# StefanHeng/ECG-Representation-Learning

Measured on AMD Instinct MI355X. Metric: 12-lead ECG records/sec pre-train step, ViT-Base bf16 @ 1/2/4/8 MI355X, higher is better.
Workload: dtype bf16

## Files before the change

### ecg-representation-learning_amd/engine.py

```python
import math
from collections import OrderedDict

import os

import torch

from . import hip
from .hip import lib, check, ptr, stream, GEMM_NT, GEMM_NN, GEMM_TN
from .hip import EPI_BIAS, EPI_GELU, EPI_GELU_BWD, EPI_RESIDUAL, EPI_DROPOUT, EPI_COLSUM, EPI_GELU_GRAD_AUX, EPI_MUL_AUX

LN_EPS = 1e-5


def _align(n, a=8):
    return (n + a - 1) // a * a


def _numel(shape):
    n = 1
    for v in shape:
        n *= v
    return n


# ... 603 lines not shown

    def _act_spec(self, B, masked, m, rows=None, N=None, mrows=None):
        T = self.dtype
        f32, u8 = torch.float32, torch.uint8
        if N is None:
            N = self.n if masked else self.N
        M, Mp = B * N, B * (N if masked else N - 1)
        if rows is not None:
            M, Mp = rows, rows - (0 if masked else B)
        d, f, h = self.d, self.f, self.h
        sp = OrderedDict()
        sp.update(patches=((Mp, self.CP), T), tok=((Mp, d), T), x0=((M, d), T))
        for i in range(self.Ly):
            l = dict(mean1=((M,), f32), rstd1=((M,), f32), xn1=((M, d), T), qkv=((M, 3 * d), T), attn=((M, d), T), x1=((M, d), T),
                     mean2=((M,), f32), rstd2=((M,), f32), xn2=((M, d), T), hpre=((M, f), u8 if self._aux8(M) else T), hact=((M, f), T), x2=((M, d), T))
            if T == torch.float32:
                l['probs'] = ((B * h * N * N,), T)
            else:
                l['lse'] = ((B * h * N,), f32)
            if self.fp8 and M >= 2048:
                l.update(xn1_8=((M * d,), u8), attn_8=((M * d,), u8), xn2_8=((M * d,), u8), hact_8=((M * f,), u8))
            for k, v in l.items():
                sp[f'L{i}.{k}'] = v
        sp.update(logits=((B, self.K), f32), xhat=((B, d), f32), hrstd=((B,), f32), loss_elem=((B, self.K), f32), loss_mean=((1,), f32),
                  dlogits=((B, self.K), f32))
        sp.update(dxa=((M, d), T), dxb=((M, d), T), dxn=((M, d), T), dqkv=((M, 3 * d), T), dattn=((M, d), T), dh=((M, f), T),
                  dtok=((Mp, d), T), dxm=((M, d), T))
        if T == torch.float32:
            sp.update(pd=((B * h * N * N,), T), dp=((B * h * N * N,), T))
        if T == torch.bfloat16 and not masked:
            sp.update({f'cls_{k}': ((B, d), T) for k in ('attn', 'x1', 'xn2', 'x2', 'dx', 'dy', 'dxn', 'dx1', 'dxm', 'dattn', 'dq')})
            sp.update(cls_hpre=((B, f), T), cls_hact=((B, f), T), cls_dh=((B, f), T), cls_lse=((B * h,), f32), cls_mean2=((B,), f32),
                      cls_rstd2=((B,), f32))
        l = lib()
        ws = max(l.ecgvit_layernorm_bwd_workspace(M, d), l.ecgvit_colsum_workspace(M, max(f, 3 * d)), 8 * ((M + 255) // 256) * f, 4096)
        if T == torch.bfloat16:
            for (mm, nn) in ((d, f), (f, d), (d, d), (3 * d, d), (d, self.CP)):
                ws = max(ws, hip.gemm_workspace_bytes(GEMM_TN, T, mm, nn, M))
        if masked:
            Rm = B * m if mrows is None else mrows
            sp.update(flag=((Mp,), u8), rows=((Rm, d), T), pred=((Rm, self.CP), T), target=((Rm, self.CP), T),
                      dpred=((Rm, self.CP), T), drows=((Rm, d), T), dmasked=((Mp, d), T), mloss=((1,), f32), l1part=((1024,), f32))
        sp['ws'] = ((ws,), u8)
        if self.fp8:
            sp['q8'] = ((M * max(f, 3 * d),), u8)
            sp['q8b'] = ((M * f,), u8)
        return sp

    def _ln_fwd(self, x, g, b, y, mean, rstd, rows, q8_site=None, y8=None):
        d = self.d
        if (self.fp8 and q8_site is not None and q8_site in self._f8_seen and rows >= 2048 and d % 256 == 0
                and d // 64 in (4, 8, 12, 16, 24, 32)):
            check(lib().ecgvit_layernorm_fwd_q8(ptr(x), ptr(g), ptr(b), None if (y8 is not None and self._only8(rows)) else ptr(y), ptr(mean), ptr(rstd), rows, d, LN_EPS,
                                                ptr(y8 if y8 is not None else self.act['q8']),
                                                ptr(self.f8_scale[q8_site:q8_site + 1]), ptr(self.f8_amax[q8_site:q8_site + 1]), stream()),
                  'layernorm_fwd_q8')
            return True
        check(lib().ecgvit_layernorm_fwd(ptr(x), ptr(g), ptr(b), ptr(y), ptr(mean), ptr(rstd), rows, d, LN_EPS,
                                         hip.code(self.dtype), stream()), 'layernorm_fwd')
        return False

    def _ln_bwd(self, dy, x, g, mean, rstd, dres, dx, dg, db, rows):
        check(lib().ecgvit_layernorm_bwd(ptr(dy), ptr(x), ptr(g), ptr(mean), ptr(rstd), ptr(dres), ptr(dx), ptr(dg), ptr(db),
                                         ptr(self.act['ws']), rows, self.d, hip.code(self.dtype), stream()), 'layernorm_bwd')

    def _ln_bwd_fused(self, dy, x, g, mean, rstd, dres, dx, dg, db, rows, dxm, dcolsum, p, seed, q8_site=None):
# ... 152 lines not shown
                    and N * 3 * d * 2 < 2 ** 31):
                check(l.ecgvit_attention_bwd_q8(ptr(L['qkv']), ptr(L['attn']), ptr(a['dattn']), ptr(L['lse']), ptr(a['dqkv']), B, N, h, dh, self.scale,
                                                ph, seed, ptr(a['q8']), ptr(self.f8_scale[site:site + 1]), ptr(self.f8_amax[site:site + 1]), st),
                      'attention_bwd_q8')
                return True
            check(l.ecgvit_attention_bwd(ptr(L['qkv']), ptr(L['attn']), ptr(a['dattn']), ptr(L['lse']), ptr(a['dqkv']), B, N, h, dh, self.scale, ph,
                                         seed, hip.BF16, st), 'attention_bwd')
        else:
            self._attn_bwd_f32(L, B, ph, seed)
        return False

    def _attention_cls_fwd(self, L, B, ph, seed):
        a, l, st = self.act, lib(), stream()
        h, dh, N = self.h, self.dh, self.T
        ntok = self.saved.get('ntok')
        if ntok is not None:
            check(l.ecgvit_attention_varlen_cls_fwd(ptr(L['qkv']), ptr(a['cls_attn']), ptr(a['cls_lse']), ptr(ntok), B, N, h, dh, self.scale, ph, seed,
                                                    st), 'attention_varlen_cls_fwd')
        else:
            check(l.ecgvit_attention_cls_fwd(ptr(L['qkv']), ptr(a['cls_attn']), ptr(a['cls_lse']), B, N, h, dh, self.scale, ph, seed,
                                             hip.code(self.dtype), st), 'attention_cls_fwd')

    def _attention_cls_bwd(self, L, B, ph, seed):
        a, l, st = self.act, lib(), stream()
        h, dh, N = self.h, self.dh, self.T
        ntok = self.saved.get('ntok')
        if ntok is not None:
            check(l.ecgvit_attention_varlen_cls_bwd(ptr(L['qkv']), ptr(a['cls_attn']), ptr(a['cls_dattn']), ptr(a['cls_lse']), ptr(a['dqkv']),
                                                    ptr(a['cls_dq']), ptr(ntok), B, N, h, dh, self.scale, ph, seed, st), 'attention_varlen_cls_bwd')
        else:
            check(l.ecgvit_attention_cls_bwd(ptr(L['qkv']), ptr(a['cls_attn']), ptr(a['cls_dattn']), ptr(a['cls_lse']), ptr(a['dqkv']), ptr(a['cls_dq']),
                                             B, N, h, dh, self.scale, ph, seed, hip.code(self.dtype), st), 'attention_cls_bwd')

    def _cls_block_fwd(self, L, X, B, ph, s0, lp):
        a, W, P = self.act, self.W, self.P32
        d, f, N = self.d, self.f, self.T
        M = B * N
        self._ln_fwd(X, P[lp + '0.norm.weight'], P[lp + '0.norm.bias'], L['xn1'], L['mean1'], L['rstd1'], M)
        wqkv = W[lp + '0.fn.to_qkv.weight']
        self._gemm(GEMM_NT, L['xn1'], wqkv, L['qkv'], M, 2 * d, d, d, d, 3 * d, b_off=d * d, c_off=d)
        self._gemm(GEMM_NT, L['xn1'], wqkv, L['qkv'], B, d, d, N * d, d, N * 3 * d)
        self._attention_cls_fwd(L, B, ph, s0 + 1)
        drop = EPI_DROPOUT if ph > 0 else 0
        self._gemm(GEMM_NT, a['cls_attn'], W[lp + '0.fn.to_out.0.weight'], a['cls_x1'], B, d, d, d, d, d, epilogue=EPI_BIAS | EPI_RESIDUAL | drop,
                   bias=P[lp + '0.fn.to_out.0.bias'], residual=X, ldr=N * d, dropout_p=ph, seed=s0 + 2, mask_row_pitch=N)
        self._ln_fwd(a['cls_x1'], P[lp + '1.norm.weight'], P[lp + '1.norm.bias'], a['cls_xn2'], a['cls_mean2'], a['cls_rstd2'], B)
        self._gemm(GEMM_NT, a['cls_xn2'], W[lp + '1.fn.net.0.weight'], a['cls_hact'], B, f, d, d, d, f,
                   epilogue=EPI_BIAS | EPI_GELU | EPI_GELU_GRAD_AUX | drop, bias=P[lp + '1.fn.net.0.bias'], aux=a['cls_hpre'], ldaux=f,
                   dropout_p=ph, seed=s0 + 3, mask_row_pitch=N)
        self._gemm(GEMM_NT, a['cls_hact'], W[lp + '1.fn.net.3.weight'], a['cls_x2'], B, d, f, f, f, d, epilogue=EPI_BIAS | EPI_RESIDUAL | drop,
                   bias=P[lp + '1.fn.net.3.bias'], residual=a['cls_x1'], ldr=d, dropout_p=ph, seed=s0 + 4, mask_row_pitch=N)
        return a['cls_x2']

    def forward(self, x, labels=None, weight=None, training=True, seed=0, want_mean=True, cls_only_last=False, lengths=None):
        return self._head_loss(self._trunk_pass(x, labels, weight, training, seed, cls_only_last, lengths), want_mean)

    def _head_loss(self, X, want_mean):
        a, sv, T = self.act, self.saved, hip.code(self.dtype)
        l, st = lib(), stream()
        B, d, rg, labels = sv['B'], self.d, sv['ragged'], sv['labels']
        pre = 'vit.'
        sv['head_pitch'] = 1 if (sv['cls_only_last'] or rg is not None) else self.N
        if rg is not None:
            check(l.ecgvit_gather_rows(ptr(X), ptr(rg.tok_off), ptr(a['cls_x2']), 1, rg.M, B, d, d, d, T, st), 'gather_rows')
            X = a['cls_x2']
        check(l.ecgvit_head_fwd(ptr(X), sv['head_pitch'], ptr(self.P32[pre + 'mlp_head.0.weight']), ptr(self.P32[pre + 'mlp_head.0.bias']),
                                ptr(self.P32[pre + 'mlp_head.1.weight']), ptr(self.P32[pre + 'mlp_head.1.bias']),
                                ptr(a['logits']), ptr(a['xhat']), ptr(a['hrstd']), B, d, self.K, LN_EPS, T, st), 'head_fwd')
        if labels is None:
            return a['logits'], None, None
        check(l.ecgvit_bce_fwd(ptr(a['logits']), ptr(labels), ptr(sv['weight']), ptr(a['loss_elem']),
                               ptr(a['loss_mean']) if want_mean else None, B * self.K, st), 'bce_fwd')
        return a['logits'], a['loss_elem'], (a['loss_mean'] if want_mean else None)

    def _trunk_pass(self, x, labels, weight, training, seed, cls_only_last, lengths):
# ... 448 lines not shown
        s0 = seed + 100 * (i + 1)
        Xin = a['x0'] if i == 0 else a['layers'][i - 1]['x2']
        dY = dXc
        if ph > 0:
            check(l.ecgvit_dropout_apply_rows(ptr(dXc), ptr(a['cls_dy']), B, d, N, ph, s0 + 4, T, st), 'dropout_apply_rows')
            dY = a['cls_dy']
        self._colsum(dY, d, G[lp + '1.fn.net.3.bias'], B, d)
        if self._wants(lp + '1.fn.net.3.weight'):
            self._gemm(GEMM_TN, dY, a['cls_hact'], G[lp + '1.fn.net.3.weight'], d, f, B, d, f, f, workspace=ws)
        b = self._stage(i, 0)
        if not self._reach(b):
            return None, None
        self._gemm(GEMM_NN, dY, W[lp + '1.fn.net.3.weight'], a['cls_dh'], B, f, d, d, f, f, epilogue=EPI_MUL_AUX | EPI_COLSUM, aux=a['cls_hpre'],
                   ldaux=f, workspace=ws, colsum_out=G[lp + '1.fn.net.0.bias'])
        if self._wants(lp + '1.fn.net.0.weight'):
            self._gemm(GEMM_TN, a['cls_dh'], a['cls_xn2'], G[lp + '1.fn.net.0.weight'], f, d, B, f, d, d, workspace=ws)
        if not self._reach(b + 1):
            return None, None
        self._gemm(GEMM_NN, a['cls_dh'], W[lp + '1.fn.net.0.weight'], a['cls_dxn'], B, d, f, f, d, d)
        if not self._reach(b + 2):
            return None, None
        check(l.ecgvit_layernorm_bwd_fused_rowpitch(ptr(a['cls_dxn']), ptr(a['cls_x1']), ptr(P[lp + '1.norm.weight']), ptr(a['cls_mean2']),
                                                    ptr(a['cls_rstd2']), ptr(dXc), ptr(a['cls_dx1']), ptr(G[lp + '1.norm.weight']),
                                                    ptr(G[lp + '1.norm.bias']), ptr(ws), B, d, ptr(a['cls_dxm']), ptr(G[lp + '0.fn.to_out.0.bias']),
                                                    ph, s0 + 2, N, T, st), 'layernorm_bwd_fused_rowpitch')
        dY = a['cls_dxm'] if ph > 0 else a['cls_dx1']
        if self._wants(lp + '0.fn.to_out.0.weight'):
            self._gemm(GEMM_TN, dY, a['cls_attn'], G[lp + '0.fn.to_out.0.weight'], d, d, B, d, d, d, workspace=ws)
        if not self._reach(b + 3):
            return None, None
        self._gemm(GEMM_NN, dY, W[lp + '0.fn.to_out.0.weight'], a['cls_dattn'], B, d, d, d, d, d)
        if not self._reach(b + 4):
            return None, None
        self._attention_cls_bwd(L, B, ph, s0 + 1)
        name = lp + '0.fn.to_qkv.weight'
        if self._wants(name):
            self._gemm(GEMM_TN, a['dqkv'], L['xn1'], G[name], 2 * d, d, M, 3 * d, d, d, workspace=ws, a_off=d, c_off=d * d)
            self._gemm(GEMM_TN, a['cls_dq'], L['xn1'], G[name], d, d, B, d, N * d, d, workspace=ws)
        if not self._reach(b + 5):
            return None, None
        wt = self.WT.get(name)
        if wt is not None and M >= 2048:
            self._gemm(GEMM_NT, a['dqkv'], wt, a['dxn'], M, d, 2 * d, 3 * d, 3 * d, d, a_off=d, b_off=d)
        else:
            self._gemm(GEMM_NN, a['dqkv'], W[name], a['dxn'], M, d, 2 * d, 3 * d, d, d, a_off=d, b_off=d * d)
        self._gemm(GEMM_NN, a['cls_dq'], W[name], a['dxn'], B, d, d, d, d, N * d, epilogue=hip.EPI_ACCUM)
        if not self._reach(b + 6):
            return None, None
        dres.zero_()
        check(l.ecgvit_scatter_rows(ptr(a['cls_dx1']), ptr(self._cls_rows(B)), ptr(dres), B, N, 1, d, d, d, T, st), 'scatter_rows')
        if i > 0:
            lq = f'vit.transformer.layers.{i - 1}.'
            self._ln_bwd_fused(a['dxn'], Xin, P[lp + '0.norm.weight'], L['mean1'], L['rstd1'], dres, out, G[lp + '0.norm.weight'],
                               G[lp + '0.norm.bias'], M, a['dxm'], G[lq + '1.fn.net.3.bias'], ph, seed + 100 * i + 4)
        else:
            self._ln_bwd(a['dxn'], Xin, P[lp + '0.norm.weight'], L['mean1'], L['rstd1'], dres, out, G[lp + '0.norm.weight'], G[lp + '0.norm.bias'], M)
        self._ready(f'layer{i}')
        return out, dres

    def _cls_rows(self, B):
        t = getattr(self, '_cls_idx', None)
        if t is None or t.numel() < B or t.device != self.device:
            t = self._cls_idx = torch.zeros(max(B, 1), dtype=torch.int32, device=self.device)
        return t[:B]

    def _attn_bwd_f32(self, L, B, ph, seed):
        d, h, dh, N = self.d, self.h, self.dh, self.T
        a = self.act
        qkv, P, dqkv, dO, dP = L['qkv'], L['probs'], a['dqkv'], a['dattn'], a['dp']
        sq, so, sp = (N * 3 * d, dh), (N * d, dh), (h * N * N, N * N)
        Pd = P
        if ph > 0:
            Pd = a['pd']
            self._drop_apply_f32(P, Pd, B * h * N * N, ph, seed)
        self._gemm(GEMM_TN, Pd, dO, dqkv, N, dh, N, N, d, 3 * d, batch=(B, h), strideA=sp, strideB=so, strideC=sq, c_off=2 * d)
# ... 65 lines not shown
```

### ecg-representation-learning_amd/hip.py

```python
import ctypes
import os
from ctypes import c_int, c_int32, c_int64, c_uint64, c_float, c_double, c_void_p, c_char_p, POINTER, Structure, byref

import torch

_PKG_DIR = os.path.dirname(os.path.abspath(__file__))
LIB_PATH = os.path.join(_PKG_DIR, 'libecgvit_hip.so')

ABI_VERSION = 6
F32, BF16, FP8_E4M3, BF8_E5M2 = 0, 1, 2, 3
GEMM_NT, GEMM_NN, GEMM_TN = 0, 1, 2
EPI_BIAS, EPI_GELU, EPI_GELU_BWD, EPI_RESIDUAL, EPI_ACCUM, EPI_DROPOUT, EPI_COLSUM = 1, 2, 4, 8, 16, 32, 64
EPI_GELU_GRAD_AUX, EPI_MUL_AUX, EPI_QUANT_OUT, EPI_NO_OUT, EPI_AUX8 = 128, 256, 512, 1024, 2048

ACC_INIT, ACC_ADD, ACC_FOLD = 0, 1, 2
KERNEL_NONE, KERNEL_GEMM_F32, KERNEL_GEMM_BF16, KERNEL_GEMM_NT, KERNEL_GEMM_WGRAD = 0, 1, 2, 3, 4
POOL_CLS, POOL_MEAN = 0, 1
FIT_TARGETS, FIT_BINS = 16, 256
DENOISE_MAX_LEN, DENOISE_MAX_TAPS = 32768, 9
DENOISE_MAX_LEN_TILED = 1 << 25
DENOISE_MAX_POINTS = 1024

_ERR = {1: 'ECGVIT_EINVAL (unsupported shape / argument)', 2: 'ECGVIT_ELAUNCH (HIP launch failure)'}

# ... 81 lines not shown
    'ecgvit_cast_bf16_to_f32': (c_int, [_P, _P, _L, _P]),
    'ecgvit_transpose_bf16_batched': (c_int, [_P, _P, _P, _I, _L, _P]),
    'ecgvit_mask_embed_finish': (c_int, [_P, _P, _P, _P, _P, _P, _I, _I, _I, _I, _I, _P]),
    'ecgvit_mask_embed_bwd': (c_int, [_P, _P, _P, _P, _P, _I, _I, _I, _I, _P]),
    'ecgvit_mask_embed_varlen_fwd': (c_int, [_P, _P, _P, _P, _P, _P, _P, _P, _I, _I, _I, _L, _I, _I, _I, _P]),
    'ecgvit_mask_embed_varlen_bwd': (c_int, [_P, _P, _P, _P, _P, _P, _P, _P, _I, _I, _I, _I, _I, _P]),
    'ecgvit_gather_rows': (c_int, [_P, _P, _P, _I, _I, _I, _L, _L, _L, _I, _P]),
    'ecgvit_scatter_rows': (c_int, [_P, _P, _P, _I, _I, _I, _L, _L, _L, _I, _P]),
    'ecgvit_l1_loss_fwd_bwd': (c_int, [_P, _P, _P, _P, _P, _P, _L, _I, _L, _I, _P]),
    'ecgvit_eval_counts': (c_int, [_P, _L, _P, _L, _L, _I, _I, _I, _P, _P]),
    'ecgvit_pool_records': (c_int, [_P, _P, _P, _P, _I, _I, _I, _I, _P, _P, _F, _I, _P]),
    'ecgvit_rollout_workspace': (c_int64, [_I, _I, _I]),
    'ecgvit_rollout_cls': (c_int, [_P, _P, _P, _P, _P, _P, _I, _I, _I, _I, _F, _I, _P]),
    'ecgvit_rollout_colsum': (c_int, [_P, _P, _P, _P, _P, _P, _P, _P, _I, _I, _I, _I, _F, _I, _P]),
    'ecgvit_rollout_finish': (c_int, [_P, _P, _I, _I, _I, _P]),
    'ecgvit_fit_workspace': (c_int64, [_I, _I]),
    'ecgvit_fit_moments': (c_int, [_P, _P, _L, _P, _I, _I, _P, _P, _P, _P]),
    'ecgvit_fit_histogram': (c_int, [_P, _P, _L, _P, _I, _I, _P, _I, _I, _P, _P]),
    'ecgvit_fit_select': (c_int, [_P, _P, _I, _I, _I, _P]),
    'ecgvit_tok_assign': (c_int, [_P, _P, _L, _P, _P, _P, _L, _I, _I, _L, _I, _I, _P, _I, _P, _P, _P, _P, _P, _P]),
    'ecgvit_tok_workspace': (c_int64, [_I, _I]),
    'ecgvit_tok_update': (c_int, [_P, _P, _L, _P, _P, _P, _L, _I, _I, _L, _I, _I, _P, _P, _I, _P, _P, _I, _P]),
    'ecgvit_tok_decode': (c_int, [_P, _P, _L, _P, _P, _P, _L, _I, _I, _L, _I, _P, _P, _P, _I, _P]),
    'ecgvit_denoise_workspace': (c_int64, [_I, _I, _I]),
    'ecgvit_filtfilt': (c_int, [_P, _P, _P, _L, _P, _I, _I, _I, _I, POINTER(c_double), POINTER(c_double), POINTER(c_double), _I, _P, _P]),
    'ecgvit_nlm_sigma': (c_int, [_P, _P, _L, _P, _I, _I, _I, _P, _P, _P]),
    'ecgvit_nlm_denoise': (c_int, [_P, _P, _P, _L, _P, _I, _I, _I, _P, _D, _I, _I, _P]),
    'ecgvit_rloess': (c_int, [_P, _P, _P, _L, _P, _I, _I, _I, _I, _I, _D, _I, _I, _I, _P, _P]),
    'ecgvit_denoise_workspace_long': (c_int64, [_I, _I, _I]),
    'ecgvit_filtfilt_long': (c_int, [_P, _P, _P, _L, _P, _I, _I, _I, _I, POINTER(c_double), POINTER(c_double), POINTER(c_double), _I, _P, _P]),
    'ecgvit_nlm_sigma_long': (c_int, [_P, _P, _L, _P, _I, _I, _I, _P, _P, _P]),
    'ecgvit_nlm_denoise_tiled': (c_int, [_P, _P, _P, _L, _P, _I, _I, _I, _P, _D, _I, _I, _I, _P]),
    'ecgvit_rloess_tiled': (c_int, [_P, _P, _P, _L, _P, _I, _I, _I, _I, _I, _D, _I, _I, _I, _P, _I, _P]),
}

_lib = None


def use_library(path):
    global LIB_PATH
    if _lib is not None:
        raise RuntimeError('use_library() must come before the first ecgvit call of the process')
    if not os.path.exists(path):
        raise HipLibraryMissing(f'{path} not found')
    LIB_PATH = os.path.abspath(path)


def lib():
    global _lib
    if _lib is None:
        if not os.path.exists(LIB_PATH):
            raise HipLibraryMissing(
                f'{LIB_PATH} not found: build it with `python -c "import __graft_entry__ as g; g.build()"` '
                f'(or `make -C {os.path.join(_PKG_DIR, "csrc")}`). There is no CPU / eager fallback.')
        l = ctypes.CDLL(LIB_PATH)
        for name, (res, args) in SIGNATURES.items():
            fn = getattr(l, name)
            fn.restype, fn.argtypes = res, args
        _lib = l
    return _lib


def check(rc, what):
    if rc != 0:
        raise RuntimeError(f'{what}: {_ERR.get(rc, rc)}')

# ... 68 lines not shown
```

### include/ecgvit_hip.h

```cpp
#ifndef ECGVIT_HIP_H
#define ECGVIT_HIP_H

#include <stdint.h>

#ifdef __cplusplus
extern "C" {
#endif

#define ECGVIT_OK 0
#define ECGVIT_EINVAL 1
#define ECGVIT_ELAUNCH 2

#define ECGVIT_F32 0
#define ECGVIT_BF16 1
#define ECGVIT_FP8_E4M3 2
#define ECGVIT_BF8_E5M2 3

const char *ecgvit_version(void);
int ecgvit_abi_version(void);

#define ECGVIT_GEMM_NT 0
#define ECGVIT_GEMM_NN 1
#define ECGVIT_GEMM_TN 2

// ... 202 lines not shown

int ecgvit_tok_assign(const float *x, const int64_t *src_off, int64_t lead_stride, const int32_t *raw_len, const int64_t *seg_cum,
                      const int64_t *dst_off, int64_t dst_stride, int R, int C, int64_t n_seg, int k, int pad, const float *centers, int V,
                      const int32_t *prev_ids, int32_t *ids, float *means, float *dist, uint64_t *changed, void *stream);
int64_t ecgvit_tok_workspace(int V, int k);
int ecgvit_tok_update(const float *x, const int64_t *src_off, int64_t lead_stride, const int32_t *raw_len, const int64_t *seg_cum,
                      const int64_t *dst_off, int64_t dst_stride, int R, int C, int64_t n_seg, int k, int pad, const int32_t *ids,
                      float *centers, int V, int64_t *lens, void *workspace, int keep_amax, void *stream);
int ecgvit_tok_decode(float *out, const int64_t *src_off, int64_t lead_stride, const int32_t *raw_len, const int64_t *seg_cum,
                      const int64_t *dst_off, int64_t dst_stride, int R, int C, int64_t n_seg, int k, const int32_t *ids, const float *means,
                      const float *centers, int V, void *stream);

int64_t ecgvit_denoise_workspace(int R, int C, int max_len);
int ecgvit_filtfilt(const float *x, float *out, const int64_t *src_off, int64_t lead_stride, const int32_t *raw_len, int R, int C, int min_len,
                    int max_len, const double *b, const double *a, const double *zi, int ntaps, void *workspace, void *stream);
int ecgvit_nlm_sigma(const float *x, const int64_t *src_off, int64_t lead_stride, const int32_t *raw_len, int R, int C, int max_len, double *sigma,
                     void *workspace, void *stream);
int ecgvit_nlm_denoise(const float *x, float *out, const int64_t *src_off, int64_t lead_stride, const int32_t *raw_len, int R, int C, int max_len,
                       const double *sigma, double scale, int patch_wd, int sch_wd, void *stream);
int ecgvit_rloess(const float *x, float *out, const int64_t *src_off, int64_t lead_stride, const int32_t *raw_len, int R, int C, int min_len,
                  int max_len, int npoints, double frac, int degree, int robust_iters, int subtract, int8_t *iters, void *stream);

int64_t ecgvit_denoise_workspace_long(int R, int C, int max_len);
int ecgvit_filtfilt_long(const float *x, float *out, const int64_t *src_off, int64_t lead_stride, const int32_t *raw_len, int R, int C, int min_len,
                         int max_len, const double *b, const double *a, const double *zi, int ntaps, void *workspace, void *stream);
int ecgvit_nlm_sigma_long(const float *x, const int64_t *src_off, int64_t lead_stride, const int32_t *raw_len, int R, int C, int max_len, double *sigma,
                          void *workspace, void *stream);
int ecgvit_nlm_denoise_tiled(const float *x, float *out, const int64_t *src_off, int64_t lead_stride, const int32_t *raw_len, int R, int C, int max_len,
                             const double *sigma, double scale, int patch_wd, int sch_wd, int tile_runs, void *stream);
int ecgvit_rloess_tiled(const float *x, float *out, const int64_t *src_off, int64_t lead_stride, const int32_t *raw_len, int R, int C, int min_len,
                        int max_len, int npoints, double frac, int degree, int robust_iters, int subtract, int8_t *iters, int tile_samples,
                        void *stream);

#ifdef __cplusplus
}
#endif
#endif
```

Measured before the change: 7110.

## Fold CLS-only last-layer K/V projections into query-side vectors to skip full K/V GEMMs

When only the CLS token is needed in the last block, the K and V projections over all tokens are no longer computed. Instead, each head's query is folded through Wk into a vector u, scores are taken directly against the normed inputs, probabilities weight the input rows, and Wv is applied afterward. The backward pass is folded the same way, and dedicated kernels compute the K/V weight gradients. This removes an M x 2d x d GEMM in the forward pass and its matching backward GEMMs, at the cost of custom fp32 MFMA kernels, extra fp32 buffers and a possible change in numerics.

```diff
diff --git a/ecg-representation-learning_amd/csrc/cls_kv_fold.hip b/ecg-representation-learning_amd/csrc/cls_kv_fold.hip
--- /dev/null
+++ b/ecg-representation-learning_amd/csrc/cls_kv_fold.hip
@@ -0,0 +1,425 @@
+#include "common.h"
+
+namespace {
+
+constexpr int CF_MAX_N = 2048;
+constexpr int CF_MAX_H = 12;
+constexpr int CF_LDS_BYTES = 64 * 1024;
+
+__host__ __device__ inline int cf_pitch(int N) {
+    const int np = (N + 15) & ~15;
+    return (np & 31) ? np : np + 16;
+}
+static inline int cf_strips(int d) { return d / 128; }
+static inline int cf_parts(int d) { return 12 / cf_strips(d); }
+
+static bool cf_shape_ok(int N, int h, int d) {
+    if (N < 1 || N > CF_MAX_N || h < 2 || h > CF_MAX_H || (h & 1) || d != 64 * h) return false;
+    return ((int64_t)h * d + 2ll * h * cf_pitch(N)) * 4 <= CF_LDS_BYTES;
+}
+
+template <bool DROP> __device__ __forceinline__ float cf_mult(uint32_t smix, uint32_t quad0, int key, uint32_t thresh, float inv_keep) {
+    if constexpr (!DROP) return 1.f;
+    const uint32_t hsh = quad_hash(smix, quad0 + (uint32_t)(key >> 2));
+    return ((hsh >> (8 * (key & 3))) & 0xFFu) >= thresh ? inv_keep : 0.f;
+}
+
+__device__ __forceinline__ f32x4 cf_mfma(float a, float b, f32x4 c) { return __builtin_amdgcn_mfma_f32_16x16x4f32(a, b, c, 0, 0, 0); }
+__device__ __forceinline__ f32x4 cf_ld4(const float *p) { return *reinterpret_cast<const f32x4 *>(p); }
+__device__ __forceinline__ void cf_st4(float *p, f32x4 v) { *reinterpret_cast<f32x4 *>(p) = v; }
+__device__ __forceinline__ void cf_unpack(u32x4 raw, float (&v)[8]) {
+#pragma unroll
+    for (int i = 0; i < 4; ++i) {
+        v[2 * i] = __uint_as_float(raw[i] << 16);
+        v[2 * i + 1] = __uint_as_float(raw[i] & 0xFFFF0000u);
+    }
+}
+
+__device__ __forceinline__ void cf_fill_frags(float *frag, const float *__restrict__ u, int h, int d) {
+    const int d4 = d >> 2;
+    for (int i = threadIdx.x; i < h * d4; i += blockDim.x) {
+        const int n = i / d4, q = i - n * d4;
+        cf_st4(frag + ((int64_t)q * h + n) * 4, cf_ld4(u + (int64_t)n * d + 4 * q));
+    }
+}
+
+__device__ __forceinline__ void cf_scores(const bf16_t *__restrict__ y, const float *frag, float *out, int np, int N, int h, int d, float mul,
+                                          int wave, int nwaves, int lane) {
+    const int r = lane & 15, kq = lane >> 4;
+    const int nn = min(r, h - 1);
+    const int steps = d >> 5;
+    for (int t = wave; t * 16 < N; t += nwaves) {
+        const bf16_t *yr = y + (int64_t)min(t * 16 + r, N - 1) * d + 8 * kq;
+        f32x4 acc = {0.f, 0.f, 0.f, 0.f};
+        u32x4 raw[4];
+#pragma unroll
+        for (int p = 0; p < 4; ++p) raw[p] = *reinterpret_cast<const u32x4 *>(yr + 32 * p);
+        for (int s = 0; s < steps; s += 4) {
+#pragma unroll
+            for (int p = 0; p < 4; ++p) {
+                const u32x4 cur = raw[p];
+                if (s + p + 4 < steps) raw[p] = *reinterpret_cast<const u32x4 *>(yr + 32 * (s + p + 4));
+                const float *fb = frag + ((int64_t)(8 * (s + p) + 2 * kq) * h + nn) * 4;
+                const f32x4 b0 = cf_ld4(fb), b1 = cf_ld4(fb + 4 * h);
+                float a[8];
+                cf_unpack(cur, a);
+#pragma unroll
+                for (int i = 0; i < 4; ++i) acc = cf_mfma(a[i], b0[i], acc);
+#pragma unroll
+                for (int i = 0; i < 4; ++i) acc = cf_mfma(a[4 + i], b1[i], acc);
+            }
+        }
+#pragma unroll
+        for (int g = 0; g < 4; ++g) {
+            const int j = t * 16 + kq * 4 + g;
+            if (r < h && j < N) out[r * np + j] = acc[g] * mul;
+        }
+    }
+}
+
+__device__ __forceinline__ void cf_weighted_rows(const bf16_t *__restrict__ y, const float *coef, int np, float *red, float *__restrict__ dst, int N,
+                                                 int h, int d, int strip, int part, int parts, int lane) {
+    const int n = lane & 15, kq = lane >> 4;
+    const int c0 = strip * 128 + 8 * n;
+    const float *ca = coef + min(n, h - 1) * np + kq;
+    const int nsteps = (N + 3) >> 2;
+    f32x4 acc[8];
+#pragma unroll
+    for (int i = 0; i < 8; ++i) acc[i] = f32x4{0.f, 0.f, 0.f, 0.f};
+    auto load = [&](int s) -> u32x4 {
+        const int row = 4 * s + kq;
+        return row < N ? *reinterpret_cast<const u32x4 *>(y + (int64_t)row * d + c0) : u32x4{0u, 0u, 0u, 0u};
+    };
+    u32x4 raw[4];
+#pragma unroll
+    for (int p = 0; p < 4; ++p) raw[p] = part + p * parts < nsteps ? load(part + p * parts) : u32x4{0u, 0u, 0u, 0u};
+    for (int s0 = part; s0 < nsteps; s0 += 4 * parts) {
+#pragma unroll
+        for (int p = 0; p < 4; ++p) {
+            const int s = s0 + p * parts;
+            if (s < nsteps) {
+                const u32x4 cur = raw[p];
+                if (s + 4 * parts < nsteps) raw[p] = load(s + 4 * parts);
+                const float a = ca[4 * s];
+                float v[8];
+                cf_unpack(cur, v);
+#pragma unroll
+                for (int i = 0; i < 8; ++i) acc[i] = cf_mfma(a, v[i], acc[i]);
+            }
+        }
+    }
+    for (int p = 0; p < parts; ++p) {
+        if (part == p) {
+#pragma unroll
+            for (int g = 0; g < 4; ++g) {
+                const int head = kq * 4 + g;
+                if (head < h) {
+                    f32x4 v0 = {acc[0][g], acc[1][g], acc[2][g], acc[3][g]}, v1 = {acc[4][g], acc[5][g], acc[6][g], acc[7][g]};
+                    float *rp = red + head * d + c0;
+                    if (p > 0) {
+                        v0 = cf_ld4(rp) + v0;
+                        v1 = cf_ld4(rp + 4) + v1;
+                    }
+                    if (p == parts - 1) {
+                        cf_st4(dst + (int64_t)head * d + c0, v0);
+                        cf_st4(dst + (int64_t)head * d + c0 + 4, v1);
+                    } else {
+                        cf_st4(rp, v0);
+                        cf_st4(rp + 4, v1);
+                    }
+                }
+            }
+        }
+        __syncthreads();
+    }
+}
+
+template <bool DROP>
+__global__ __launch_bounds__(768) void cls_fold_fwd_kernel(const bf16_t *__restrict__ xn, const float *__restrict__ u, float *__restrict__ probs,
+                                                          float *__restrict__ t, int N, int h, int d, int parts, float scale, uint64_t seed,
+                                                          uint32_t thresh, float inv_keep) {
+    extern __shared__ __attribute__((aligned(16))) float cf_smem[];
+    const int np = cf_pitch(N);
+    float *frag = cf_smem, *sc = cf_smem + h * d;
+    const int b = blockIdx.x;
+    const int lane = threadIdx.x & 63, wave = __builtin_amdgcn_readfirstlane(threadIdx.x >> 6), nwaves = blockDim.x >> 6;
+    const bf16_t *y = xn + (int64_t)b * N * d;
+    cf_fill_frags(frag, u + (int64_t)b * h * d, h, d);
+    __syncthreads();
+    cf_scores(y, frag, sc, np, N, h, d, scale, wave, nwaves, lane);
+    __syncthreads();
+    const uint32_t smix = seed_mix(seed);
+    for (int head = wave; head < h; head += nwaves) {
+        float *s = sc + head * np;
+        float m = -INFINITY;
+        for (int j = lane; j < N; j += 64) m = fmaxf(m, s[j]);
+        m = wave_max(m);
+        float sum = 0.f;
+        for (int j = lane; j < N; j += 64) sum += __expf(s[j] - m);
+        const float l = m + __logf(wave_sum(sum));
+        const uint32_t quad0 = (uint32_t)(b * h + head) * (uint32_t)N * (uint32_t)((N + 3) >> 2);
+        float *pr = probs + ((int64_t)b * h + head) * N;
+        for (int j = lane; j < np; j += 64) {
+            float pd = 0.f;
+            if (j < N) {
+                const float p = __expf(s[j] - l);
+                pr[j] = p;
+                pd = p * cf_mult<DROP>(smix, quad0, j, thresh, inv_keep);
+            }
+            s[j] = pd;
+        }
+    }
+    __syncthreads();
+    cf_weighted_rows(y, sc, np, frag, t + (int64_t)b * h * d, N, h, d, wave % (d >> 7), wave / (d >> 7), parts, lane);
+}
+
+template <bool DROP>
+__global__ __launch_bounds__(768) void cls_fold_bwd_kernel(const bf16_t *__restrict__ xn, const float *__restrict__ u, const float *__restrict__ w,
+                                                          const float *__restrict__ probs, float *__restrict__ z, bf16_t *__restrict__ dxn, int N,
+                                                          int h, int d, int parts, float scale, uint64_t seed, uint32_t thresh, float inv_keep) {
+    extern __shared__ __attribute__((aligned(16))) float cf_smem[];
+    const int np = cf_pitch(N);
+    float *frag = cf_smem, *coef = cf_smem + h * d;
+    const int b = blockIdx.x;
+    const int lane = threadIdx.x & 63, wave = __builtin_amdgcn_readfirstlane(threadIdx.x >> 6), nwaves = blockDim.x >> 6;
+    const bf16_t *y = xn + (int64_t)b * N * d;
+    const float *ub = u + (int64_t)b * h * d, *wb = w + (int64_t)b * h * d;
+    cf_fill_frags(frag, wb, h, d);
+    __syncthreads();
+    cf_scores(y, frag, coef, np, N, h, d, 1.0f, wave, nwaves, lane);
+    __syncthreads();
+    const uint32_t smix = seed_mix(seed);
+    for (int head = wave; head < h; head += nwaves) {
+        float *dp = coef + head * np, *pdr = coef + (h + head) * np;
+        const float *pr = probs + ((int64_t)b * h + head) * N;
+        const uint32_t quad0 = (uint32_t)(b * h + head) * (uint32_t)N * (uint32_t)((N + 3) >> 2);
+        float D = 0.f;
+        for (int j = lane; j < N; j += 64) D = fmaf(pr[j] * cf_mult<DROP>(smix, quad0, j, thresh, inv_keep), dp[j], D);
+        D = wave_sum(D);
+        for (int j = lane; j < np; j += 64) {
+            float ds = 0.f, pd = 0.f;
+            if (j < N) {
+                const float p = pr[j], mlt = cf_mult<DROP>(smix, quad0, j, thresh, inv_keep);
+                pd = p * mlt;
+                ds = scale * p * (dp[j] * mlt - D);
+            }
+            dp[j] = ds;
+            pdr[j] = pd;
+        }
+    }
+    __syncthreads();
+    const int strips = d >> 7, strip = wave % strips, part = wave / strips;
+    cf_weighted_rows(y, coef, np, frag, z + (int64_t)b * h * d, N, h, d, strip, part, parts, lane);
+    if (dxn == nullptr) return;
+    const int n = lane & 15, kq = lane >> 4, ksteps = h >> 1;
+    const int c0 = strip * 128 + 8 * n;
+    f32x4 bf[CF_MAX_H / 2][2];
+#pragma unroll
+    for (int ks = 0; ks < CF_MAX_H / 2; ++ks) {
+        bf[ks][0] = bf[ks][1] = f32x4{0.f, 0.f, 0.f, 0.f};
+        if (ks < ksteps) {
+            const int kk = 4 * ks + kq;
+            const float *src = (kk < h ? ub + (int64_t)kk * d : wb + (int64_t)(kk - h) * d) + c0;
+            bf[ks][0] = cf_ld4(src);
+            bf[ks][1] = cf_ld4(src + 4);
+        }
+    }
+    bf16_t *dy = dxn + (int64_t)b * N * d + c0;
+    for (int t = part; t * 16 < N; t += parts) {
+        f32x4 acc[8];
+#pragma unroll
+        for (int i = 0; i < 8; ++i) acc[i] = f32x4{0.f, 0.f, 0.f, 0.f};
+#pragma unroll
+        for (int ks = 0; ks < CF_MAX_H / 2; ++ks) {
+            if (ks < ksteps) {
+                const float a = coef[(4 * ks + kq) * np + t * 16 + n];
+#pragma unroll
+                for (int i = 0; i < 8; ++i) acc[i] = cf_mfma(a, bf[ks][i >> 2][i & 3], acc[i]);
+            }
+        }
+#pragma unroll
+        for (int g = 0; g < 4; ++g) {
+            const int row = t * 16 + kq * 4 + g;
+            if (row < N) {
+                bf16x8 o;
+#pragma unroll
+                for (int i = 0; i < 8; ++i) o[i] = (bf16_t)acc[i][g];
+                *reinterpret_cast<bf16x8 *>(dy + (int64_t)row * d) = o;
+            }
+        }
+    }
+}
+
+__global__ __launch_bounds__(128) void cls_fold_vec_kernel(const bf16_t *__restrict__ x, int64_t ldx, const bf16_t *__restrict__ W,
+                                                          float *__restrict__ out, int B, int h, int d) {
+    __shared__ __attribute__((aligned(16))) float xs[64][16];
+    const int head = blockIdx.y, b0 = blockIdx.z * 16, c = blockIdx.x * 256 + 2 * threadIdx.x;
+    for (int i = threadIdx.x; i < 1024; i += 128) {
+        const int bb = i >> 6, e = i & 63;
+        xs[e][bb] = b0 + bb < B ? (float)x[(int64_t)(b0 + bb) * ldx + 64 * head + e] : 0.f;
+    }
+    __syncthreads();
+    if (c >= d) return;
+    float a0[16], a1[16];
+#pragma unroll
+    for (int k = 0; k < 16; ++k) a0[k] = a1[k] = 0.f;
+    const bf16_t *wp = W + (int64_t)64 * head * d + c;
+#pragma unroll 4
+    for (int e = 0; e < 64; ++e) {
+        const bf16x2 wv = *reinterpret_cast<const bf16x2 *>(wp + (int64_t)e * d);
+        const float w0 = (float)wv[0], w1 = (float)wv[1];
+#pragma unroll
+        for (int q = 0; q < 4; ++q) {
+            const f32x4 xv = cf_ld4(&xs[e][4 * q]);
+#pragma unroll
+            for (int k = 0; k < 4; ++k) {
+                a0[4 * q + k] = fmaf(xv[k], w0, a0[4 * q + k]);
+                a1[4 * q + k] = fmaf(xv[k], w1, a1[4 * q + k]);
+            }
+        }
+    }
+#pragma unroll
+    for (int k = 0; k < 16; ++k)
+        if (b0 + k < B) *reinterpret_cast<f32x2 *>(out + ((int64_t)(b0 + k) * h + head) * d + c) = f32x2{a0[k], a1[k]};
+}
+
+__global__ __launch_bounds__(256) void cls_fold_head_kernel(const float *__restrict__ v, const bf16_t *__restrict__ W, bf16_t *__restrict__ out,
+                                                           int64_t ldo, int B, int h, int d) {
+    extern __shared__ __attribute__((aligned(16))) float cf_smem[];
+    const int head = blockIdx.x, b0 = blockIdx.y * 16, d4 = d >> 2;
+    for (int i = threadIdx.x; i < 16 * d4; i += 256) {
+        const int bb = i / d4, q = i - bb * d4;
+        cf_st4(cf_smem + bb * d + 4 * q, b0 + bb < B ? cf_ld4(v + ((int64_t)(b0 + bb) * h + head) * d + 4 * q) : f32x4{0.f, 0.f, 0.f, 0.f});
+    }
+    __syncthreads();
+    const int e = threadIdx.x & 63, wv = threadIdx.x >> 6;
+    const bf16_t *wp = W + (int64_t)(64 * head + e) * d;
+    float acc[4] = {0.f, 0.f, 0.f, 0.f};
+#pragma unroll 2
+    for (int c = 0; c < d; c += 8) {
+        float wf[8];
+        cf_unpack(*reinterpret_cast<const u32x4 *>(wp + c), wf);
+#pragma unroll
+        for (int k = 0; k < 4; ++k) {
+            const float *tp = cf_smem + (4 * wv + k) * d + c;
+            const f32x4 t0 = cf_ld4(tp), t1 = cf_ld4(tp + 4);
+#pragma unroll
+            for (int i = 0; i < 4; ++i) acc[k] = fmaf(wf[i], t0[i], acc[k]);
+#pragma unroll
+            for (int i = 0; i < 4; ++i) acc[k] = fmaf(wf[4 + i], t1[i], acc[k]);
+        }
+    }
+#pragma unroll
+    for (int k = 0; k < 4; ++k)
+        if (b0 + 4 * wv + k < B) out[(int64_t)(b0 + 4 * wv + k) * ldo + 64 * head + e] = (bf16_t)acc[k];
+}
+
+__global__ __launch_bounds__(512) void cls_fold_wgrad_kernel(const bf16_t *__restrict__ xk, int64_t ldk, const float *__restrict__ vk,
+                                                            float *__restrict__ dWk, const bf16_t *__restrict__ xv, int64_t ldv,
+                                                            const float *__restrict__ vv, float *__restrict__ dWv, int B, int h, int d) {
+    __shared__ float red[16][64];
+    const bool vside = blockIdx.z >= 4;
+    const bf16_t *x = vside ? xv : xk;
+    const int64_t ldx = vside ? ldv : ldk;
+    const float *v = vside ? vv : vk;
+    float *dW = vside ? dWv : dWk;
+    const int head = blockIdx.y, e0 = 16 * (blockIdx.z & 3), lane = threadIdx.x & 63, c = blockIdx.x * 64 + lane;
+    const int wave = __builtin_amdgcn_readfirstlane(threadIdx.x >> 6);
+    float acc[16];
+#pragma unroll
+    for (int k = 0; k < 16; ++k) acc[k] = 0.f;
+#pragma unroll 4
+    for (int b = wave; b < B; b += 8) {
+        const float vc = v[((int64_t)b * h + head) * d + c];
+        const bf16_t *xp = x + (int64_t)b * ldx + 64 * head + e0;
+        float xf[16];
+        cf_unpack(*reinterpret_cast<const u32x4 *>(xp), *reinterpret_cast<float(*)[8]>(xf));
+        cf_unpack(*reinterpret_cast<const u32x4 *>(xp + 8), *reinterpret_cast<float(*)[8]>(xf + 8));
+#pragma unroll
+        for (int k = 0; k < 16; ++k) acc[k] = fmaf(xf[k], vc, acc[k]);
+    }
+    for (int p = 0; p < 8; ++p) {
+        if (wave == p) {
+#pragma unroll
+            for (int k = 0; k < 16; ++k) {
+                const float s = p > 0 ? red[k][lane] + acc[k] : acc[k];
+                if (p == 7) dW[(int64_t)(64 * head + e0 + k) * d + c] = s;
+                else red[k][lane] = s;
+            }
+        }
+        __syncthreads();
+    }
+}
+
+static bool cf_aligned16(const void *p) { return reinterpret_cast<uintptr_t>(p) % 16 == 0; }
+
+}
+
+extern "C" {
+
+int ecgvit_cls_fold_supported(int N, int h, int d) { return cf_shape_ok(N, h, d) ? 1 : 0; }
+
+int ecgvit_cls_fold_vec(const void *x, int64_t ldx, const void *W, float *out, int B, int h, int d, void *stream) {
+    if (!x || !W || !out || B < 1 || h < 1 || d != 64 * h || ldx < d || (B + 15) / 16 > 65535 || h > 65535) return ECGVIT_EINVAL;
+    hipLaunchKernelGGL(cls_fold_vec_kernel, dim3((unsigned)((d + 255) / 256), (unsigned)h, (unsigned)((B + 15) / 16)), dim3(128), 0, as_stream(stream),
+                       (const bf16_t *)x, ldx, (const bf16_t *)W, out, B, h, d);
+    ECGVIT_CHECK_LAUNCH();
+    return ECGVIT_OK;
+}
+
+int ecgvit_cls_fold_head(const float *v, const void *W, void *out, int64_t ldo, int B, int h, int d, void *stream) {
+    if (!v || !W || !out || B < 1 || h < 1 || d != 64 * h || ldo < d || 16ll * d * 4 > CF_LDS_BYTES || (B + 15) / 16 > 65535 || !cf_aligned16(v) ||
+        !cf_aligned16(W))
+        return ECGVIT_EINVAL;
+    hipLaunchKernelGGL(cls_fold_head_kernel, dim3((unsigned)h, (unsigned)((B + 15) / 16)), dim3(256), (size_t)16 * d * 4, as_stream(stream), v,
+                       (const bf16_t *)W, (bf16_t *)out, ldo, B, h, d);
+    ECGVIT_CHECK_LAUNCH();
+    return ECGVIT_OK;
+}
+
+int ecgvit_cls_fold_fwd(const void *xn, const float *u, float *probs, float *t, int B, int N, int h, int d, float scale, float dropout_p, uint64_t seed,
+                        void *stream) {
+    if (!xn || !u || !probs || !t || B < 1 || !cf_shape_ok(N, h, d) || !cf_aligned16(xn) || !cf_aligned16(u) || !cf_aligned16(t)) return ECGVIT_EINVAL;
+    if (dropout_p > 0.f && dropout_threshold8(dropout_p) == 0) return ECGVIT_EINVAL;
+    const uint32_t th = dropout_threshold8(dropout_p);
+    const float ik = dropout_inv_keep8(dropout_p);
+    const int parts = cf_parts(d);
+    const dim3 grid((unsigned)B), block((unsigned)(64 * cf_strips(d) * parts));
+    const size_t lds = ((size_t)h * d + (size_t)h * cf_pitch(N)) * 4;
+    const bf16_t *y = (const bf16_t *)xn;
+    if (th) hipLaunchKernelGGL(cls_fold_fwd_kernel<true>, grid, block, lds, as_stream(stream), y, u, probs, t, N, h, d, parts, scale, seed, th, ik);
+    else hipLaunchKernelGGL(cls_fold_fwd_kernel<false>, grid, block, lds, as_stream(stream), y, u, probs, t, N, h, d, parts, scale, seed, th, ik);
+    ECGVIT_CHECK_LAUNCH();
+    return ECGVIT_OK;
+}
+
+int ecgvit_cls_fold_bwd(const void *xn, const float *u, const float *w, const float *probs, float *z, void *dxn, int B, int N, int h, int d,
+                        float scale, float dropout_p, uint64_t seed, void *stream) {
+    if (!xn || !u || !w || !probs || !z || B < 1 || !cf_shape_ok(N, h, d) || !cf_aligned16(xn) || !cf_aligned16(u) || !cf_aligned16(w) ||
+        !cf_aligned16(z) || !cf_aligned16(dxn))
+        return ECGVIT_EINVAL;
+    if (dropout_p > 0.f && dropout_threshold8(dropout_p) == 0) return ECGVIT_EINVAL;
+    const uint32_t th = dropout_threshold8(dropout_p);
+    const float ik = dropout_inv_keep8(dropout_p);
+    const int parts = cf_parts(d);
+    const dim3 grid((unsigned)B), block((unsigned)(64 * cf_strips(d) * parts));
+    const size_t lds = ((size_t)h * d + 2 * (size_t)h * cf_pitch(N)) * 4;
+    const bf16_t *y = (const bf16_t *)xn;
+    if (th) hipLaunchKernelGGL(cls_fold_bwd_kernel<true>, grid, block, lds, as_stream(stream), y, u, w, probs, z, (bf16_t *)dxn, N, h, d, parts, scale, seed, th, ik);
+    else hipLaunchKernelGGL(cls_fold_bwd_kernel<false>, grid, block, lds, as_stream(stream), y, u, w, probs, z, (bf16_t *)dxn, N, h, d, parts, scale, seed, th, ik);
+    ECGVIT_CHECK_LAUNCH();
+    return ECGVIT_OK;
+}
+
+int ecgvit_cls_fold_wgrad(const void *q0, int64_t ldq, const float *z, float *dWk, const void *dout, int64_t lddo, const float *t, float *dWv, int B,
+                          int h, int d, void *stream) {
+    if (!q0 || !z || !dWk || !dout || !t || !dWv || B < 1 || h < 1 || h > 65535 || d != 64 * h || ldq < d || lddo < d || (ldq & 7) || (lddo & 7) ||
+        !cf_aligned16(q0) || !cf_aligned16(dout))
+        return ECGVIT_EINVAL;
+    hipLaunchKernelGGL(cls_fold_wgrad_kernel, dim3((unsigned)(d / 64), (unsigned)h, 8), dim3(512), 0, as_stream(stream), (const bf16_t *)q0, ldq, z, dWk,
+                       (const bf16_t *)dout, lddo, t, dWv, B, h, d);
+    ECGVIT_CHECK_LAUNCH();
+    return ECGVIT_OK;
+}
+
+}
diff --git a/ecg-representation-learning_amd/engine.py b/ecg-representation-learning_amd/engine.py
--- a/ecg-representation-learning_amd/engine.py
+++ b/ecg-representation-learning_amd/engine.py
@@ -659,6 +659,8 @@
             sp.update({f'cls_{k}': ((B, d), T) for k in ('attn', 'x1', 'xn2', 'x2', 'dx', 'dy', 'dxn', 'dx1', 'dxm', 'dattn', 'dq')})
             sp.update(cls_hpre=((B, f), T), cls_hact=((B, f), T), cls_dh=((B, f), T), cls_lse=((B * h,), f32), cls_mean2=((B,), f32),
                       cls_rstd2=((B,), f32))
+            sp.update({f'cls_{k}': ((B, h, d), f32) for k in ('u', 'w', 't', 'z')})
+            sp['cls_p'] = ((B * h * N,), f32)
         l = lib()
         ws = max(l.ecgvit_layernorm_bwd_workspace(M, d), l.ecgvit_colsum_workspace(M, max(f, 3 * d)), 8 * ((M + 255) // 256) * f, 4096)
         if T == torch.bfloat16:
@@ -877,15 +879,44 @@
             check(l.ecgvit_attention_cls_bwd(ptr(L['qkv']), ptr(a['cls_attn']), ptr(a['cls_dattn']), ptr(a['cls_lse']), ptr(a['dqkv']), ptr(a['cls_dq']),
                                              B, N, h, dh, self.scale, ph, seed, hip.code(self.dtype), st), 'attention_cls_bwd')
 
+    cls_kv_fold = True
+
+    def _fold_kv(self):
+        sv = self.saved
+        return (self.cls_kv_fold and self.dtype == torch.bfloat16 and not self.fp8 and self.dh == 64 and sv.get('ntok') is None
+                and sv.get('ragged') is None and bool(lib().ecgvit_cls_fold_supported(self.T, self.h, self.d)))
+
+    def _cls_fold_fwd(self, L, wqkv, B, ph, seed):
+        a, l, st = self.act, lib(), stream()
+        d, h, N = self.d, self.h, self.T
+        wk, wv = wqkv[d:], wqkv[2 * d:]
+        check(l.ecgvit_cls_fold_vec(ptr(L['qkv']), N * 3 * d, ptr(wk), ptr(a['cls_u']), B, h, d, st), 'cls_fold_vec')
+        check(l.ecgvit_cls_fold_fwd(ptr(L['xn1']), ptr(a['cls_u']), ptr(a['cls_p']), ptr(a['cls_t']), B, N, h, d, self.scale, ph, seed, st),
+              'cls_fold_fwd')
+        check(l.ecgvit_cls_fold_head(ptr(a['cls_t']), ptr(wv), ptr(a['cls_attn']), d, B, h, d, st), 'cls_fold_head')
+
+    def _cls_fold_bwd(self, L, wqkv, B, ph, seed, want_dxn):
+        a, l, st = self.act, lib(), stream()
+        d, h, N = self.d, self.h, self.T
+        wk, wv = wqkv[d:], wqkv[2 * d:]
+        check(l.ecgvit_cls_fold_vec(ptr(a['cls_dattn']), d, ptr(wv), ptr(a['cls_w']), B, h, d, st), 'cls_fold_vec')
+        check(l.ecgvit_cls_fold_bwd(ptr(L['xn1']), ptr(a['cls_u']), ptr(a['cls_w']), ptr(a['cls_p']), ptr(a['cls_z']),
+                                    ptr(a['dxn']) if want_dxn else None, B, N, h, d, self.scale, ph, seed, st), 'cls_fold_bwd')
+        check(l.ecgvit_cls_fold_head(ptr(a['cls_z']), ptr(wk), ptr(a['cls_dq']), d, B, h, d, st), 'cls_fold_head')
+
     def _cls_block_fwd(self, L, X, B, ph, s0, lp):
         a, W, P = self.act, self.W, self.P32
         d, f, N = self.d, self.f, self.T
         M = B * N
         self._ln_fwd(X, P[lp + '0.norm.weight'], P[lp + '0.norm.bias'], L['xn1'], L['mean1'], L['rstd1'], M)
         wqkv = W[lp + '0.fn.to_qkv.weight']
-        self._gemm(GEMM_NT, L['xn1'], wqkv, L['qkv'], M, 2 * d, d, d, d, 3 * d, b_off=d * d, c_off=d)
-        self._gemm(GEMM_NT, L['xn1'], wqkv, L['qkv'], B, d, d, N * d, d, N * 3 * d)
-        self._attention_cls_fwd(L, B, ph, s0 + 1)
+        if self._fold_kv():
+            self._gemm(GEMM_NT, L['xn1'], wqkv, L['qkv'], B, d, d, N * d, d, N * 3 * d)
+            self._cls_fold_fwd(L, wqkv, B, ph, s0 + 1)
+        else:
+            self._gemm(GEMM_NT, L['xn1'], wqkv, L['qkv'], M, 2 * d, d, d, d, 3 * d, b_off=d * d, c_off=d)
+            self._gemm(GEMM_NT, L['xn1'], wqkv, L['qkv'], B, d, d, N * d, d, N * 3 * d)
+            self._attention_cls_fwd(L, B, ph, s0 + 1)
         drop = EPI_DROPOUT if ph > 0 else 0
         self._gemm(GEMM_NT, a['cls_attn'], W[lp + '0.fn.to_out.0.weight'], a['cls_x1'], B, d, d, d, d, d, epilogue=EPI_BIAS | EPI_RESIDUAL | drop,
                    bias=P[lp + '0.fn.to_out.0.bias'], residual=X, ldr=N * d, dropout_p=ph, seed=s0 + 2, mask_row_pitch=N)
@@ -1400,15 +1431,25 @@
         self._gemm(GEMM_NN, dY, W[lp + '0.fn.to_out.0.weight'], a['cls_dattn'], B, d, d, d, d, d)
         if not self._reach(b + 4):
             return None, None
-        self._attention_cls_bwd(L, B, ph, s0 + 1)
         name = lp + '0.fn.to_qkv.weight'
+        fold = self._fold_kv()
+        if fold:
+            self._cls_fold_bwd(L, W[name], B, ph, s0 + 1, self._reach(b + 5))
+        else:
+            self._attention_cls_bwd(L, B, ph, s0 + 1)
         if self._wants(name):
-            self._gemm(GEMM_TN, a['dqkv'], L['xn1'], G[name], 2 * d, d, M, 3 * d, d, d, workspace=ws, a_off=d, c_off=d * d)
+            if fold:
+                check(l.ecgvit_cls_fold_wgrad(ptr(L['qkv']), N * 3 * d, ptr(a['cls_z']), ptr(G[name][d:]), ptr(a['cls_dattn']), d, ptr(a['cls_t']),
+                                              ptr(G[name][2 * d:]), B, self.h, d, st), 'cls_fold_wgrad')
+            else:
+                self._gemm(GEMM_TN, a['dqkv'], L['xn1'], G[name], 2 * d, d, M, 3 * d, d, d, workspace=ws, a_off=d, c_off=d * d)
             self._gemm(GEMM_TN, a['cls_dq'], L['xn1'], G[name], d, d, B, d, N * d, d, workspace=ws)
         if not self._reach(b + 5):
             return None, None
         wt = self.WT.get(name)
-        if wt is not None and M >= 2048:
+        if fold:
+            pass
+        elif wt is not None and M >= 2048:
             self._gemm(GEMM_NT, a['dqkv'], wt, a['dxn'], M, d, 2 * d, 3 * d, 3 * d, d, a_off=d, b_off=d)
         else:
             self._gemm(GEMM_NN, a['dqkv'], W[name], a['dxn'], M, d, 2 * d, 3 * d, d, d, a_off=d, b_off=d * d)
diff --git a/ecg-representation-learning_amd/hip.py b/ecg-representation-learning_amd/hip.py
--- a/ecg-representation-learning_amd/hip.py
+++ b/ecg-representation-learning_amd/hip.py
@@ -137,6 +137,12 @@
     'ecgvit_nlm_sigma_long': (c_int, [_P, _P, _L, _P, _I, _I, _I, _P, _P, _P]),
     'ecgvit_nlm_denoise_tiled': (c_int, [_P, _P, _P, _L, _P, _I, _I, _I, _P, _D, _I, _I, _I, _P]),
     'ecgvit_rloess_tiled': (c_int, [_P, _P, _P, _L, _P, _I, _I, _I, _I, _I, _D, _I, _I, _I, _P, _I, _P]),
+    'ecgvit_cls_fold_supported': (c_int, [_I, _I, _I]),
+    'ecgvit_cls_fold_vec': (c_int, [_P, _L, _P, _P, _I, _I, _I, _P]),
+    'ecgvit_cls_fold_head': (c_int, [_P, _P, _P, _L, _I, _I, _I, _P]),
+    'ecgvit_cls_fold_fwd': (c_int, [_P, _P, _P, _P, _I, _I, _I, _I, _F, _F, _U, _P]),
+    'ecgvit_cls_fold_bwd': (c_int, [_P, _P, _P, _P, _P, _P, _I, _I, _I, _I, _F, _F, _U, _P]),
+    'ecgvit_cls_fold_wgrad': (c_int, [_P, _L, _P, _P, _P, _L, _P, _P, _I, _I, _I, _P]),
 }
 
 _lib = None
diff --git a/include/ecgvit_hip.h b/include/ecgvit_hip.h
--- a/include/ecgvit_hip.h
+++ b/include/ecgvit_hip.h
@@ -258,6 +258,16 @@
                         int max_len, int npoints, double frac, int degree, int robust_iters, int subtract, int8_t *iters, int tile_samples,
                         void *stream);
 
+int ecgvit_cls_fold_supported(int N, int h, int d);
+int ecgvit_cls_fold_vec(const void *x, int64_t ldx, const void *W, float *out, int B, int h, int d, void *stream);
+int ecgvit_cls_fold_head(const float *v, const void *W, void *out, int64_t ldo, int B, int h, int d, void *stream);
+int ecgvit_cls_fold_fwd(const void *xn, const float *u, float *probs, float *t, int B, int N, int h, int d, float scale, float dropout_p,
+                        uint64_t seed, void *stream);
+int ecgvit_cls_fold_bwd(const void *xn, const float *u, const float *w, const float *probs, float *z, void *dxn, int B, int N, int h, int d,
+                        float scale, float dropout_p, uint64_t seed, void *stream);
+int ecgvit_cls_fold_wgrad(const void *q0, int64_t ldq, const float *z, float *dWk, const void *dout, int64_t lddo, const float *t, float *dWv,
+                          int B, int h, int d, void *stream);
+
 #ifdef __cplusplus
 }
 #endif
```

New measurement: 7164, median of 6. No clear change (+0.8%).
